# flavie-yuan-liu/DL_attack_on_ImageNet

Hardware: AMD Instinct MI355X
Metric: adversarial images/sec (ADiL learning step, classifier included) (higher is better)
Workload: dtype bf16; 1 GPU; ADiL learn_dictionary_a step vs resnet50, 512 images/GPU, 50 atoms, 224x224, bf16 image streams + fp32 D/V master, loss=logits, clean pseudo-labels computed once per image and cached (1 fwd + 1 bwd per step; result-neutral, profiles/r03_label_stability.md); global_batch=512, atoms=50, inner_iters=131, parallelism=dp1: images+codes sharded, D replicated, 1 all-reduce(grad_d)/step

## Files before the change

### dl_attack_on_imagenet_amd/_lib.py

```python
import ctypes
import os
from ctypes import c_float, c_int, c_size_t, c_void_p

_PKG = os.path.dirname(os.path.abspath(__file__))
LIBPATH = os.environ.get("ADIL_HIP_LIBRARY") or os.path.join(_PKG, "lib", "libadil_hip.so")

SIGNATURES = {
    "adil_abi_version": (c_int, []),
    "adil_max_atoms": (c_int, []),
    "adil_grad_workspace_bytes": (c_size_t, [c_int, c_int, c_int]),
    "adil_grad_code_rows": (c_int, [c_int]),
    "adil_grad_slab_offset": (c_size_t, [c_int, c_int, c_int]),
    "adil_pack_codes": (c_int, [c_void_p, c_void_p, c_int, c_int, c_void_p, c_void_p, c_void_p, c_int, c_void_p, c_int, c_int,
                                c_void_p]),
    "adil_gather_images": (c_int, [c_void_p, c_int, c_void_p, c_void_p, c_int, c_int, c_int, c_void_p]),
    "adil_spd_inverse": (c_int, [c_void_p, c_int, c_void_p, c_void_p]),
    "adil_synth": (c_int, [c_void_p, c_void_p, c_void_p, c_void_p, c_int, c_int, c_int, c_int, c_float, c_int, c_void_p]),
    "adil_images_to_u8": (c_int, [c_void_p, c_int, c_void_p, c_size_t, c_void_p, c_void_p]),
    "adil_synth_store": (c_int, [c_void_p, c_void_p, c_void_p, c_void_p, c_void_p, c_int, c_int, c_int, c_int, c_float, c_int,
                                 c_void_p]),
    "adil_synth_fp8": (c_int, [c_void_p, c_void_p, c_void_p, c_void_p, c_int, c_int, c_int, c_int, c_float, c_float, c_int,
                               c_void_p]),
    "adil_dict_to_fp8": (c_int, [c_void_p, c_size_t, c_void_p, c_void_p]),
    "adil_adamw_clamp_fp8": (c_int, [c_void_p, c_void_p, c_int, c_void_p, c_void_p, c_size_t, c_float, c_float, c_float,
# ... 15 lines not shown
                                  c_float, c_float, c_float, c_float, c_float, c_void_p, c_void_p, c_float, c_void_p, c_void_p,
                                  c_void_p, c_int, c_int, c_void_p]),
    "adil_atom_l1ball_project": (c_int, [c_void_p, c_int, c_int, c_int, c_float, c_void_p]),
    "adil_l1ball_project": (c_int, [c_void_p, c_int, c_int, c_float, c_void_p]),
    "adil_l2ball_project": (c_int, [c_void_p, c_int, c_int, c_float, c_void_p]),
    "adil_ista_step": (c_int, [c_void_p, c_void_p, c_size_t, c_float, c_float, c_void_p]),
    "adil_atom_workspace_bytes": (c_size_t, [c_int, c_int]),
    "adil_atom_norms": (c_int, [c_void_p, c_int, c_int, c_void_p, c_void_p, c_size_t, c_void_p]),
    "adil_atom_scale": (c_int, [c_void_p, c_int, c_int, c_void_p, c_int, c_void_p]),
    "adil_gram_workspace_bytes": (c_size_t, [c_int, c_int]),
    "adil_gram": (c_int, [c_void_p, c_int, c_int, c_void_p, c_void_p, c_size_t, c_void_p]),
    "adil_dict_rightmul": (c_int, [c_void_p, c_void_p, c_int, c_int, c_void_p, c_void_p]),
    "adil_image_metrics": (c_int, [c_void_p, c_void_p, c_int, c_int, c_int, c_void_p, c_void_p, c_void_p]),
    "adil_affine_act_fwd": (c_int, [c_void_p, c_void_p, c_void_p, c_void_p, c_void_p, c_size_t, c_int, c_int, c_int, c_int,
                                    c_void_p]),
    "adil_affine_act_bwd": (c_int, [c_void_p, c_void_p, c_void_p, c_void_p, c_void_p, c_size_t, c_int, c_int, c_int, c_int,
                                    c_void_p]),
    "adil_stem_conv_fwd": (c_int, [c_void_p, c_int, c_void_p, c_float, c_float, c_float, c_float, c_float, c_float,
                                   c_void_p, c_void_p, c_void_p, c_int, c_int, c_int, c_void_p]),
    "adil_maxpool_fwd": (c_int, [c_void_p, c_void_p, c_void_p, c_int, c_int, c_int, c_int, c_void_p]),
    "adil_stem_pool_bwd": (c_int, [c_void_p, c_void_p, c_void_p, c_void_p, c_void_p, c_int, c_int, c_int, c_int, c_void_p]),
    "adil_pw_conv_fwd": (c_int, [c_void_p, c_void_p, c_void_p, c_void_p, c_void_p, c_void_p, c_int, c_int, c_int, c_int,
                                 c_void_p, c_void_p, c_int, c_int, c_void_p]),
    "adil_pw_conv_bwd": (c_int, [c_void_p, c_void_p, c_void_p, c_void_p, c_void_p, c_void_p, c_void_p, c_int, c_int, c_int,
                                 c_int, c_void_p, c_void_p, c_void_p, c_void_p, c_int, c_int, c_void_p]),
    "adil_pw_conv_bwd_tile": (c_int, [c_void_p, c_void_p, c_void_p, c_void_p, c_void_p, c_void_p, c_void_p, c_int, c_int, c_int,
                                      c_int, c_void_p, c_void_p, c_void_p, c_void_p, c_int, c_int, c_void_p, c_int]),
    "adil_pw_route_policy": (c_int, [c_int]),
    "adil_pw_join_fwd": (c_int, [c_void_p, c_void_p, c_void_p, c_void_p, c_void_p, c_void_p, c_void_p, c_void_p, c_void_p,
                                 c_void_p, c_void_p, c_void_p, c_int, c_int, c_int, c_void_p]),
    "adil_pw_join_bwd": (c_int, [c_void_p, c_void_p, c_void_p, c_void_p, c_void_p, c_void_p, c_void_p, c_void_p, c_void_p,
                                 c_void_p, c_void_p, c_void_p, c_void_p, c_int, c_int, c_int, c_void_p]),
    "adil_conv3x3": (c_int, [c_void_p, c_void_p, c_void_p, c_int, c_int, c_int, c_int, c_int, c_void_p]),
    "adil_conv3x3_s2_fwd": (c_int, [c_void_p, c_void_p, c_void_p, c_int, c_int, c_int, c_int, c_int, c_void_p]),
    "adil_conv3x3_s2_bwd": (c_int, [c_void_p, c_void_p, c_void_p, c_int, c_int, c_int, c_int, c_int, c_void_p]),
    "adil_dw3x3_fwd": (c_int, [c_void_p, c_void_p, c_void_p, c_void_p, c_int, c_int, c_int, c_int, c_int, c_int, c_void_p]),
    "adil_dw3x3_bwd": (c_int, [c_void_p, c_void_p, c_void_p, c_void_p, c_int, c_int, c_int, c_int, c_int, c_int, c_void_p]),
    "adil_pw8_fwd": (c_int, [c_void_p, c_void_p, c_void_p, c_void_p, c_void_p, c_void_p, c_int, c_int, c_int, c_int, c_void_p]),
    "adil_pw8_bwd": (c_int, [c_void_p, c_void_p, c_void_p, c_void_p, c_void_p, c_int, c_int, c_int, c_int, c_void_p]),
    "adil_stem_conv_bwd": (c_int, [c_void_p, c_void_p, c_float, c_float, c_float, c_void_p, c_int, c_int, c_int, c_int,
                                   c_void_p]),
    "adil_first3x3_fwd": (c_int, [c_void_p, c_int, c_void_p, c_float, c_float, c_float, c_float, c_float, c_float,
                                  c_void_p, c_void_p, c_void_p, c_int, c_int, c_int, c_int, c_void_p]),
    "adil_first3x3_bwd": (c_int, [c_void_p, c_void_p, c_void_p, c_void_p, c_float, c_float, c_float, c_void_p, c_int, c_int,
                                  c_int, c_int, c_int, c_void_p]),
    "adil_pool_head_fwd": (c_int, [c_void_p, c_void_p, c_void_p, c_void_p, c_void_p, c_int, c_int, c_int, c_int, c_void_p]),
    "adil_pool_head_bwd": (c_int, [c_void_p, c_void_p, c_void_p, c_void_p, c_int, c_int, c_int, c_int, c_void_p]),
    "adil_dense1x1_fwd": (c_int, [c_void_p, c_void_p, c_void_p, c_void_p, c_void_p, c_void_p, c_void_p, c_int, c_int, c_int,
                                  c_int, c_void_p]),
    "adil_dense1x1_bwd": (c_int, [c_void_p, c_void_p, c_void_p, c_void_p, c_void_p, c_void_p, c_void_p, c_void_p, c_int, c_int,
                                  c_int, c_int, c_void_p]),
    "adil_dense3x3_fwd": (c_int, [c_void_p, c_void_p, c_void_p, c_int, c_int, c_int, c_int, c_int, c_void_p]),
    "adil_dense3x3_bwd": (c_int, [c_void_p, c_void_p, c_void_p, c_int, c_int, c_int, c_int, c_int, c_void_p]),
    "adil_dense1x1_fwd_ld": (c_int, [c_void_p, c_int, c_void_p, c_void_p, c_void_p, c_void_p, c_void_p, c_void_p, c_int, c_int,
                                     c_int, c_int, c_int, c_void_p]),
    "adil_dense1x1_bwd_ld": (c_int, [c_void_p, c_int, c_void_p, c_int, c_void_p, c_void_p, c_void_p, c_int, c_void_p, c_void_p,
                                     c_void_p, c_int, c_int, c_int, c_int, c_int, c_int, c_void_p]),
    "adil_dense3x3_fwd_ld": (c_int, [c_void_p, c_int, c_void_p, c_void_p, c_int, c_int, c_int, c_int, c_int, c_int, c_void_p]),
    "adil_dense3x3_bwd_ld": (c_int, [c_void_p, c_int, c_void_p, c_void_p, c_int, c_int, c_int, c_int, c_int, c_int, c_void_p]),
    "adil_dense_transition_fwd": (c_int, [c_void_p, c_void_p, c_void_p, c_void_p, c_void_p, c_int, c_int, c_int, c_int, c_int,
                                          c_void_p]),
    "adil_dense_transition_bwd": (c_int, [c_void_p, c_int, c_void_p, c_void_p, c_void_p, c_void_p, c_void_p, c_int, c_int,
                                          c_int, c_int, c_int, c_void_p]),
}

ABI_VERSION = 8
# ... 39 lines not shown
```

### dl_attack_on_imagenet_amd/csrc/adil_convs.hip

```cpp
#include <hip/hip_runtime.h>
#include <stdint.h>

#include "adil_common.h"
#include "adil_hip.h"
#include "adil_mfma.h"

namespace {

#define PW_BM 128
#define PW_BK 64
#define PW_LS (PW_BK + 8)
#define PW_PK 512

template <int BN, bool PRO, bool RES>
__global__ __launch_bounds__(256) __attribute__((amdgpu_waves_per_eu(PRO && BN == 128 ? 2 : (RES ? 3 : 4)))) void pw_conv_fwd_kernel(
    const bf16_t* __restrict__ x, const bf16_t* __restrict__ wgt, const float* __restrict__ scale,
    const float* __restrict__ shift, const bf16_t* __restrict__ res, bf16_t* __restrict__ y, int M, int K, int N,
    int relu, int MT, int NT, const float* __restrict__ pscale, const float* __restrict__ pshift, int sub_w, int sub_hw) {
    constexpr int CT = BN / 32;
    constexpr int XCH = PW_BM * PW_BK / 8 / 256;
    constexpr int WCH = BN * PW_BK / 8 / 256;
    constexpr int OS = BN + 8;
    extern __shared__ __attribute__((aligned(16))) unsigned char smem_raw[];
    bf16_t* sx = reinterpret_cast<bf16_t*>(smem_raw);
// ... 715 lines not shown

}

extern "C" int adil_pw_join_fwd(const void* h2raw, const float* pscale2, const float* pshift2, const void* w3,
                                const float* scale3, const float* shift3, const void* res, void* out, const void* w1,
                                const float* scale1, const float* shift1, void* h1, int M, int W, int C, void* stream) {
    ADIL_ENTER();
    if (!h2raw || !pscale2 || !pshift2 || !w3 || !scale3 || !shift3 || !res || !out || !w1 || !scale1 || !shift1 || !h1 ||
        M <= 0 || (W != 64 && W != 128) || C != 4 * W)
        return ADIL_EINVAL;
    const JoinArgs a = {(const bf16_t*)h2raw, nullptr, pscale2, pshift2, (const bf16_t*)w3, scale3, shift3,
                        (const bf16_t*)res, nullptr, (bf16_t*)out, (const bf16_t*)w1, scale1, shift1, nullptr, (bf16_t*)h1,
                        M, C};
    return launch_pw_join_w<false>(a, W, (hipStream_t)stream);
}

extern "C" int adil_pw_join_bwd(const void* g_h1, const void* h1, const float* scale1, const void* wt1, const void* g_out,
                                const void* out, const float* scale3, void* gres, const void* wt3, const void* h2raw,
                                const float* pscale2, const float* pshift2, void* gx, int M, int W, int C, void* stream) {
    ADIL_ENTER();
    if (!g_h1 || !h1 || !scale1 || !wt1 || !g_out || !out || !scale3 || !gres || !wt3 || !h2raw || !pscale2 || !pshift2 ||
        !gx || M <= 0 || (W != 64 && W != 128) || C != 4 * W)
        return ADIL_EINVAL;
    const JoinArgs a = {(const bf16_t*)g_h1, (const bf16_t*)h1, scale1, nullptr, (const bf16_t*)wt1, scale3, nullptr,
                        (const bf16_t*)g_out, (const bf16_t*)out, (bf16_t*)gres, (const bf16_t*)wt3, pscale2, pshift2,
                        (const bf16_t*)h2raw, (bf16_t*)gx, M, C};
    return launch_pw_join_w<true>(a, W, (hipStream_t)stream);
}

namespace {

#define C3_LS 72

template <int BN, int WPX>
__global__ __launch_bounds__(256) __attribute__((amdgpu_waves_per_eu(2))) void conv3x3_kernel(
    const bf16_t* __restrict__ x, const bf16_t* __restrict__ wp, bf16_t* __restrict__ y, int M, int H, int W, int C, int N,
    int MT, int NT) {
    constexpr int C3_BM = WPX * 64;
    constexpr int CTW = BN / 32 / (4 / WPX);
    constexpr int XCHK = (C3_BM + 128) * 8 / 256;
    constexpr int WCH = BN * 8 / 256;
    constexpr int OS = BN + 8;
    extern __shared__ __attribute__((aligned(16))) unsigned char smem_raw[];
    const int NP = C3_BM + 2 * W + 2;
    bf16_t* sx = reinterpret_cast<bf16_t*>(smem_raw);
    const int sx_elems = (NP * C3_LS > C3_BM * OS ? NP * C3_LS : C3_BM * OS);
    bf16_t* sw = sx + ((sx_elems + 7) & ~7);
    const int tid = threadIdx.x, lane = tid & 63, w = tid >> 6, c = lane & 31, h = lane >> 5;
    const int wpx = w % WPX, wch = w / WPX;
    int mt, nt;
    if ((MT & 7) == 0) {
        const int xcd = blockIdx.x & 7, j = blockIdx.x >> 3;
        nt = j % NT;
        mt = (j / NT) * 8 + xcd;
    } else {
        nt = blockIdx.x % NT;
        mt = blockIdx.x / NT;
    }
    const int m0 = mt * C3_BM, n0 = nt * BN;
    const int nci = C >> 6;

    int pl[2];
    unsigned vmask[2];
#pragma unroll
    for (int p = 0; p < 2; ++p) {
        pl[p] = (wpx * 2 + p) * 32 + c;
        const int m = m0 + pl[p];
        const int ww = m % W, hh = (m / W) % H;
        unsigned vm = 0;
#pragma unroll
        for (int t = 0; t < 9; ++t) {
            const int kh = t / 3, kw = t - 3 * kh;
            const bool ok = (m < M) && (hh + kh - 1 >= 0) && (hh + kh - 1 < H) && (ww + kw - 1 >= 0) && (ww + kw - 1 < W);
            vm |= ok ? (1u << t) : 0u;
        }
        vmask[p] = vm;
    }

    u32x4 xr[XCHK], wr[3][WCH];
    auto load_x = [&](int cc) {
#pragma unroll
        for (int i = 0; i < XCHK; ++i) {
            const int q = tid + 256 * i, px = q >> 3, ch = q & 7;
            int gm = m0 - W - 1 + (px < NP ? px : NP - 1);
            gm = gm < 0 ? 0 : (gm >= M ? M - 1 : gm);
            xr[i] = *reinterpret_cast<const u32x4*>(x + (size_t)gm * C + cc * 64 + ch * 8);
        }
    };
    auto store_x = [&]() {
#pragma unroll
        for (int i = 0; i < XCHK; ++i) {
            const int q = tid + 256 * i, px = q >> 3, ch = q & 7;
            if (px < NP) *reinterpret_cast<u32x4*>(sx + px * C3_LS + ch * 8) = xr[i];
        }
    };
    const int nit = nci * 9;
    auto load_w = [&](int it, u32x4 (&r)[WCH]) {
        const int itc = it < nit ? it : nit - 1;
        const int cc = itc / 9, tap = itc - 9 * cc;
#pragma unroll
        for (int i = 0; i < WCH; ++i) {
            const int q = tid + 256 * i, row = q >> 3, ch = q & 7;
            r[i] = *reinterpret_cast<const u32x4*>(wp + ((size_t)(n0 + row) * 9 + tap) * C + cc * 64 + ch * 8);
        }
    };
    auto store_w = [&](int buf, const u32x4 (&r)[WCH]) {
#pragma unroll
        for (int i = 0; i < WCH; ++i) {
            const int q = tid + 256 * i, row = q >> 3, ch = q & 7;
            *reinterpret_cast<u32x4*>(sw + (buf * BN + row) * C3_LS + ch * 8) = r[i];
        }
    };

    f32x16 acc[2][CTW];
#pragma unroll
    for (int p = 0; p < 2; ++p)
#pragma unroll
        for (int ct = 0; ct < CTW; ++ct)
#pragma unroll
            for (int r = 0; r < 16; ++r) acc[p][ct][r] = 0.0f;

    auto tap_body = [&](int it, u32x4 (&rfree)[WCH], const u32x4 (&rnext)[WCH]) {
        const int buf = it & 1;
        const int cc = it / 9, tap = it - 9 * cc;
        const int kh = tap / 3, kw = tap - 3 * kh;
        load_w(it + 3, rfree);
        if (tap == 4 && cc + 1 < nci) load_x(cc + 1);
        const bf16_t* bw = sw + (buf * BN + (wch * CTW) * 32 + c) * C3_LS + 8 * h;
        const int shift = kh * W + kw;
        const bool ok0 = (vmask[0] >> tap) & 1u, ok1 = (vmask[1] >> tap) & 1u;
#pragma unroll
        for (int ks = 0; ks < 4; ++ks) {
            bf16x8 b0 = lds8(sx + (pl[0] + shift) * C3_LS + 16 * ks + 8 * h);
            bf16x8 b1 = lds8(sx + (pl[1] + shift) * C3_LS + 16 * ks + 8 * h);
            u32x4 z0 = __builtin_bit_cast(u32x4, b0), z1 = __builtin_bit_cast(u32x4, b1);
#pragma unroll
            for (int j = 0; j < 4; ++j) { z0[j] = ok0 ? z0[j] : 0u; z1[j] = ok1 ? z1[j] : 0u; }
            b0 = __builtin_bit_cast(bf16x8, z0);
            b1 = __builtin_bit_cast(bf16x8, z1);
#pragma unroll
            for (int ct = 0; ct < CTW; ++ct) {
                const bf16x8 a = lds8(bw + ct * 32 * C3_LS + 16 * ks);
                mma16(acc[0][ct], a, b0);
                mma16(acc[1][ct], a, b1);
            }
        }
        if (it + 1 < nit) store_w(buf ^ 1, rnext);
        if (tap == 8 && cc + 1 < nci) {
            lds_barrier();
            store_x();
        }
        lds_barrier();
    };

    load_x(0);
    load_w(0, wr[0]);
    load_w(1, wr[1]);
    load_w(2, wr[2]);
    store_x();
    store_w(0, wr[0]);
    __syncthreads();
    for (int it = 0; it < nit; it += 3) {
        tap_body(it, wr[0], wr[1]);
        tap_body(it + 1, wr[1], wr[2]);
        tap_body(it + 2, wr[2], wr[0]);
    }
#pragma unroll
    for (int p = 0; p < 2; ++p) {
#pragma unroll
        for (int ct = 0; ct < CTW; ++ct) {
#pragma unroll
            for (int q = 0; q < 4; ++q) {
                u32x2 t;
                t[0] = pack2_bf16(acc[p][ct][4 * q], acc[p][ct][4 * q + 1]);
                t[1] = pack2_bf16(acc[p][ct][4 * q + 2], acc[p][ct][4 * q + 3]);
                *reinterpret_cast<u32x2*>(sx + pl[p] * OS + (wch * CTW + ct) * 32 + 8 * q + 4 * h) = t;
            }
        }
    }
    __syncthreads();
    constexpr int CPP = BN / 8;
#pragma unroll
    for (int i = 0; i < C3_BM * CPP / 256; ++i) {
        const int id = tid + 256 * i, px = id / CPP, ch = id - px * CPP;
        const int mm = m0 + px;
        if (mm < M) *reinterpret_cast<u32x4*>(y + (size_t)mm * N + n0 + ch * 8) = *reinterpret_cast<const u32x4*>(sx + px * OS + ch * 8);
    }
}

template <int BN, int WPX>
int launch_conv3x3(const void* x, const void* wp, void* y, int M, int H, int W, int C, int N, hipStream_t st) {
    constexpr int C3_BM = WPX * 64;
    const int MT = (M + C3_BM - 1) / C3_BM, NT = N / BN;
    const int NP = C3_BM + 2 * W + 2;
    size_t sx_elems = (size_t)NP * C3_LS;
    if (sx_elems < (size_t)C3_BM * (BN + 8)) sx_elems = (size_t)C3_BM * (BN + 8);
    sx_elems = (sx_elems + 7) & ~(size_t)7;
    const size_t lds = (sx_elems + (size_t)2 * BN * C3_LS) * sizeof(bf16_t);
    if (lds > 160 * 1024) return ADIL_EINVAL;
    if (lds > 48 * 1024) {
        const hipError_t e = hipFuncSetAttribute((const void*)conv3x3_kernel<BN, WPX>, hipFuncAttributeMaxDynamicSharedMemorySize,
                                                 (int)lds);
        if (e != hipSuccess) return (int)e;
    }
    hipLaunchKernelGGL((conv3x3_kernel<BN, WPX>), dim3((unsigned)(MT * NT)), dim3(256), lds, st, (const bf16_t*)x,
                       (const bf16_t*)wp, (bf16_t*)y, M, H, W, C, N, MT, NT);
    ADIL_CHECK_LAUNCH();
    return 0;
}

}

extern "C" int adil_conv3x3(const void* x, const void* wp, void* y, int B, int H, int W, int C, int N, void* stream) {
    ADIL_ENTER();
    if (!x || !wp || !y || B <= 0 || H <= 0 || W <= 0 || C <= 0 || N <= 0 || (C % 64) || (N % 64) || W > 63) return ADIL_EINVAL;
    const long long M = (long long)B * H * W;
    if (M > 0x7fffffffLL) return ADIL_EINVAL;
    if (N % 128 == 0) return launch_conv3x3<128, 2>(x, wp, y, (int)M, H, W, C, N, (hipStream_t)stream);
    return launch_conv3x3<64, 4>(x, wp, y, (int)M, H, W, C, N, (hipStream_t)stream);
}

namespace {

#define S2_BM 128

template <int BN, bool BWD>
__global__ __launch_bounds__(256) __attribute__((amdgpu_waves_per_eu(2))) void conv3x3_s2_kernel(
    const bf16_t* __restrict__ src, const bf16_t* __restrict__ wp, bf16_t* __restrict__ dst, int M, int OH, int OW, int K,
    int NO, int MT, int NT) {
    constexpr int CTW = BN / 64;
    constexpr int XCH = S2_BM * 8 / 256;
    constexpr int WCH = BN * 8 / 256;
    constexpr int OS = BN + 8;
    constexpr int PAIR = (S2_BM + BN) * C3_LS;
    constexpr int NCLS = BWD ? 4 : 1;
    static_assert(S2_BM * OS <= PAIR, "the output transpose goes through one idle buffer");
    extern __shared__ __attribute__((aligned(16))) unsigned char smem_raw[];
    bf16_t* sb = reinterpret_cast<bf16_t*>(smem_raw);
    const int tid = threadIdx.x, lane = tid & 63, w = tid >> 6, c = lane & 31, h = lane >> 5;
    const int wpx = w & 1, wch = w >> 1;
    int mt, nt;
    if ((MT & 7) == 0) {
        const int xcd = blockIdx.x & 7, j = blockIdx.x >> 3;
        nt = j % NT;
        mt = (j / NT) * 8 + xcd;
    } else {
        nt = blockIdx.x % NT;
        mt = blockIdx.x / NT;
    }
    const int m0 = mt * S2_BM, n0 = nt * BN;
    const int nci = K >> 6;
    const int nit = nci * 9;
    auto cls_ph = [](int cls) { return BWD ? (cls < 2 ? 1 : 0) : 0; };
    auto cls_pw = [](int cls) { return BWD ? ((cls & 1) ? 0 : 1) : 0; };

    int ctr[XCH];
    unsigned flg[XCH];
#pragma unroll
    for (int i = 0; i < XCH; ++i) {
        const int r = m0 + (tid >> 3) + 32 * i;
        const int rc = r < M ? r : M - 1;
        const int j = rc % OW, ii = (rc / OW) % OH;
        ctr[i] = BWD ? rc : 4 * rc - 2 * j;
        const bool okh = BWD ? (ii + 1 < OH) : (ii > 0), okw = BWD ? (j + 1 < OW) : (j > 0);
        flg[i] = (r < M ? 1u : 0u) | (okh ? 2u : 0u) | (okw ? 4u : 0u);
    }
    struct Tile {
        u32x4 x[XCH], w[WCH];
        unsigned ok;
    };
    int lcls = 0, lcc = 0, la = 0, lb = 0;
    int lph = cls_ph(0), lpw = cls_pw(0), lnth = BWD ? 1 + lph : 3, lntw = BWD ? 1 + lpw : 3;
    auto load_tiles = [&](Tile& t) {
        const int kh = BWD ? (lph ? 2 * la : 1) : la, kw = BWD ? (lpw ? 2 * lb : 1) : lb;
        const int off = BWD ? (kh == 0 ? OW : 0) + (kw == 0 ? 1 : 0) : (kh - 1) * 2 * OW + (kw - 1);
        const unsigned need = 1u | (kh == 0 ? 2u : 0u) | (kw == 0 ? 4u : 0u);
        unsigned okm = 0;
#pragma unroll
        for (int i = 0; i < XCH; ++i) {
            const int ch = tid & 7;
            const bool ok = (flg[i] & need) == need;
            okm |= ok ? (1u << i) : 0u;
            const int srow = ok ? ctr[i] + off : ctr[i];
            t.x[i] = *reinterpret_cast<const u32x4*>(src + (size_t)srow * K + lcc * 64 + ch * 8);
        }
        t.ok = okm;
#pragma unroll
        for (int i = 0; i < WCH; ++i) {
            const int q = tid + 256 * i, row = q >> 3, ch = q & 7;
            t.w[i] = *reinterpret_cast<const u32x4*>(wp + ((size_t)(n0 + row) * 9 + kh * 3 + kw) * K + lcc * 64 + ch * 8);
        }
        if (++lb == lntw) {
            lb = 0;
            if (++la == lnth) {
                la = 0;
                if (++lcc == nci && lcls + 1 < NCLS) {
                    lcc = 0;
                    ++lcls;
                    lph = cls_ph(lcls);
                    lpw = cls_pw(lcls);
                    lnth = 1 + lph;
                    lntw = 1 + lpw;
                }
            }
        }
    };
    auto store_tiles = [&](int buf, const Tile& t) {
        bf16_t* sx = sb + buf * PAIR;
        bf16_t* sw = sx + S2_BM * C3_LS;
#pragma unroll
        for (int i = 0; i < XCH; ++i) {
            const int row = (tid >> 3) + 32 * i, ch = tid & 7;
            u32x4 v = t.x[i];
            const bool ok = (t.ok >> i) & 1u;
#pragma unroll
            for (int j = 0; j < 4; ++j) v[j] = ok ? v[j] : 0u;
            *reinterpret_cast<u32x4*>(sx + row * C3_LS + ch * 8) = v;
        }
#pragma unroll
        for (int i = 0; i < WCH; ++i) {
            const int q = tid + 256 * i, row = q >> 3, ch = q & 7;
            *reinterpret_cast<u32x4*>(sw + row * C3_LS + ch * 8) = t.w[i];
        }
    };
// ... 11 lines not shown
    auto finish_class = [&](int cls, bf16_t* so) {
#pragma unroll
        for (int p = 0; p < 2; ++p) {
            const int pl = wpx * 64 + p * 32 + c;
#pragma unroll
            for (int ct = 0; ct < CTW; ++ct) {
#pragma unroll
                for (int q = 0; q < 4; ++q) {
                    u32x2 t;
                    t[0] = pack2_bf16(acc[p][ct][4 * q], acc[p][ct][4 * q + 1]);
                    t[1] = pack2_bf16(acc[p][ct][4 * q + 2], acc[p][ct][4 * q + 3]);
                    *reinterpret_cast<u32x2*>(so + pl * OS + (wch * CTW + ct) * 32 + 8 * q + 4 * h) = t;
                }
            }
        }
        lds_barrier();
        const int ph = cls_ph(cls), pw = cls_pw(cls);
        constexpr int CPP = BN / 8;
#pragma unroll
        for (int i = 0; i < S2_BM * CPP / 256; ++i) {
            const int id = tid + 256 * i, px = id / CPP, ch = id - px * CPP;
            const int r = m0 + px;
            if (r < M) {
                const size_t drow = BWD ? (size_t)(4 * r - 2 * (r % OW) + ph * 2 * OW + pw) : (size_t)r;
                *reinterpret_cast<u32x4*>(dst + drow * NO + n0 + ch * 8) = *reinterpret_cast<const u32x4*>(so + px * OS + ch * 8);
            }
        }
        lds_barrier();
        zero_acc();
    };

    int ccls = 0;
    int crem = nci * (BWD ? 4 : 9);
    auto tap_body = [&](int it, Tile& tfree, const Tile& tnext) {
        const int buf = it & 1;
        if (it + 3 < nit) load_tiles(tfree);
        const bf16_t* bx = sb + buf * PAIR + (wpx * 64 + c) * C3_LS + 8 * h;
        const bf16_t* bw = sb + buf * PAIR + (S2_BM + wch * CTW * 32 + c) * C3_LS + 8 * h;
#pragma unroll
        for (int ks = 0; ks < 4; ++ks) {
            const bf16x8 b0 = lds8(bx + 16 * ks);
            const bf16x8 b1 = lds8(bx + 32 * C3_LS + 16 * ks);
#pragma unroll
            for (int ct = 0; ct < CTW; ++ct) {
                const bf16x8 a = lds8(bw + ct * 32 * C3_LS + 16 * ks);
                mma16(acc[0][ct], a, b0);
                mma16(acc[1][ct], a, b1);
            }
        }
        if (--crem == 0) {
            finish_class(ccls, sb + (buf ^ 1) * PAIR);
            ++ccls;
            crem = nci * (1 + cls_ph(ccls)) * (1 + cls_pw(ccls));
        }
        if (it + 1 < nit) store_tiles(buf ^ 1, tnext);
        lds_barrier();
    };

    Tile t0, t1, t2;
    load_tiles(t0);
    load_tiles(t1);
    load_tiles(t2);
    store_tiles(0, t0);
    lds_barrier();
    for (int it = 0; it < nit; it += 3) {
        tap_body(it, t0, t1);
        tap_body(it + 1, t1, t2);
        tap_body(it + 2, t2, t0);
    }
}

template <int BN, bool BWD>
int launch_conv3x3_s2(const void* src, const void* wp, void* dst, int M, int OH, int OW, int K, int NO, hipStream_t st) {
    const int MT = (M + S2_BM - 1) / S2_BM, NT = NO / BN;
    const size_t lds = (size_t)2 * (S2_BM + BN) * C3_LS * sizeof(bf16_t);
    if (lds > 48 * 1024) {
        const hipError_t e = hipFuncSetAttribute((const void*)conv3x3_s2_kernel<BN, BWD>,
                                                 hipFuncAttributeMaxDynamicSharedMemorySize, (int)lds);
        if (e != hipSuccess) return (int)e;
    }
    hipLaunchKernelGGL((conv3x3_s2_kernel<BN, BWD>), dim3((unsigned)(MT * NT)), dim3(256), lds, st,
                       (const bf16_t*)src, (const bf16_t*)wp, (bf16_t*)dst, M, OH, OW, K, NO, MT, NT);
    ADIL_CHECK_LAUNCH();
    return 0;
}

bool conv3x3_s2_covers(int B, int H, int W, int C, int N, int* M) {
    if (B <= 0 || H <= 0 || W <= 0 || C <= 0 || N <= 0 || (H & 1) || (W & 1) || (C % 64) || (N % 64) || W > ADIL_CONV3X3_S2_MAX_W)
        return false;
    const long long m4 = (long long)B * H * W;
    if (m4 > 0x7fffffffLL) return false;
    *M = (int)(m4 / 4);
    return true;
}

}

extern "C" int adil_conv3x3_s2_fwd(const void* x, const void* wp, void* y, int B, int H, int W, int C, int N, void* stream) {
    ADIL_ENTER();
    int M = 0;
    if (!x || !wp || !y || !conv3x3_s2_covers(B, H, W, C, N, &M)) return ADIL_EINVAL;
    if (N % 128 == 0) return launch_conv3x3_s2<128, false>(x, wp, y, M, H / 2, W / 2, C, N, (hipStream_t)stream);
    return launch_conv3x3_s2<64, false>(x, wp, y, M, H / 2, W / 2, C, N, (hipStream_t)stream);
}

extern "C" int adil_conv3x3_s2_bwd(const void* g, const void* wp_bwd, void* gx, int B, int H, int W, int C, int N, void* stream) {
    ADIL_ENTER();
    int M = 0;
    if (!g || !wp_bwd || !gx || !conv3x3_s2_covers(B, H, W, C, N, &M)) return ADIL_EINVAL;
    if (C % 128 == 0) return launch_conv3x3_s2<128, true>(g, wp_bwd, gx, M, H / 2, W / 2, N, C, (hipStream_t)stream);
    return launch_conv3x3_s2<64, true>(g, wp_bwd, gx, M, H / 2, W / 2, N, C, (hipStream_t)stream);
}
```

### dl_attack_on_imagenet_amd/ops.py

```python
from __future__ import annotations

import math
from ctypes import byref, c_int, c_void_p
from dataclasses import dataclass
from typing import Optional, Tuple

import torch

from . import _lib

Tensor = torch.Tensor
_DTYPE_CODE = {torch.float32: 0, torch.bfloat16: 1}
ADIL_U8 = 2
_workspaces = {}


def _round_up(x: int, m: int) -> int:
    return (x + m - 1) // m * m


def stream_dtype_code(dtype: torch.dtype) -> int:
    try:
        return _DTYPE_CODE[dtype]
    except KeyError:
# ... 780 lines not shown
    @staticmethod
    def backward(ctx, g):
        lib = _lib.load()
        (wp_bwd,) = ctx.saved_tensors
        (c,) = ctx.meta
        g2 = _nhwc_grad(g)
        b, h, w, n = g2.shape
        gx = torch.empty((b, h, w, c), dtype=torch.bfloat16, device=g2.device)
        if b > 0:
            _lib.check(lib.adil_conv3x3(_ptr(g2), _ptr(wp_bwd), _ptr(gx), b, h, w, n, c, _stream()), "adil_conv3x3")
        return gx.permute(0, 3, 1, 2), None, None


def conv3x3(x: Tensor, wp_fwd: Tensor, wp_bwd: Tensor) -> Tensor:
    return Conv3x3Function.apply(x, wp_fwd, wp_bwd)


CONV3X3_S2_MAX_W = 63


def pack_conv3x3_s2_weights(weight: Tensor) -> Tuple[Tensor, Tensor]:
    n, c, kh, kw = weight.shape
    if (kh, kw) != (3, 3):
        raise ValueError(f"expected a 3x3 convolution weight, got {tuple(weight.shape)}")
    w = weight.detach().float()
    fwd = w.permute(0, 2, 3, 1).reshape(n, 9 * c).to(torch.bfloat16).contiguous()
    bwd = w.permute(1, 2, 3, 0).reshape(c, 9 * n).to(torch.bfloat16).contiguous()
    return fwd, bwd


def conv3x3_s2_covers(x: Tensor, cin: int, cout: int) -> bool:
    return (x.dim() == 4 and x.is_cuda and x.dtype == torch.bfloat16 and x.shape[1] == cin and cin % 64 == 0
            and cout % 64 == 0 and x.shape[2] % 2 == 0 and x.shape[3] % 2 == 0 and 0 < x.shape[3] <= CONV3X3_S2_MAX_W
            and x.shape[2] > 0 and x.shape[0] * x.shape[2] * x.shape[3] < 2 ** 31)


class Conv3x3S2Function(torch.autograd.Function):

    @staticmethod
    def forward(ctx, x, wp_fwd, wp_bwd):
        lib = _lib.load()
        b, c, h, w = x.shape
        n = wp_fwd.shape[0]
        x2 = _nhwc(x)
        y = torch.empty((b, h // 2, w // 2, n), dtype=torch.bfloat16, device=x.device)
        if b > 0:
            _lib.check(lib.adil_conv3x3_s2_fwd(_ptr(x2), _ptr(wp_fwd), _ptr(y), b, h, w, c, n, _stream()),
                       "adil_conv3x3_s2_fwd")
        ctx.save_for_backward(wp_bwd)
        ctx.meta = (c, h, w)
        return y.permute(0, 3, 1, 2)

    @staticmethod
    def backward(ctx, g):
        lib = _lib.load()
        (wp_bwd,) = ctx.saved_tensors
        c, h, w = ctx.meta
        g2 = _nhwc_grad(g)
        b, n = g2.shape[0], g2.shape[3]
        gx = torch.empty((b, h, w, c), dtype=torch.bfloat16, device=g2.device)
        if b > 0:
            _lib.check(lib.adil_conv3x3_s2_bwd(_ptr(g2), _ptr(wp_bwd), _ptr(gx), b, h, w, c, n, _stream()),
                       "adil_conv3x3_s2_bwd")
        return gx.permute(0, 3, 1, 2), None, None


def conv3x3_s2(x: Tensor, wp_fwd: Tensor, wp_bwd: Tensor) -> Tensor:
# ... 594 lines not shown
```

### include/adil_hip.h

```cpp
#ifndef ADIL_HIP_H
#define ADIL_HIP_H

#include <stddef.h>
#include <stdint.h>

#ifdef __cplusplus
extern "C" {
#endif

#define ADIL_F32 0
#define ADIL_BF16 1
#define ADIL_U8 2

#define ADIL_EINVAL (-1)
#define ADIL_EWORKSPACE (-2)

int adil_abi_version(void);

int adil_max_atoms(void);

size_t adil_grad_workspace_bytes(int B, int P, int K);

int adil_grad_code_rows(int K);

// ... 61 lines not shown
size_t adil_gram_workspace_bytes(int P, int K);
int adil_gram(const float* d, int P, int K, float* gram, void* ws, size_t ws_bytes, void* stream);

int adil_spd_inverse(const float* a, int K, float* out, void* stream);

int adil_dict_rightmul(const float* d, const float* mat, int P, int K, float* out, void* stream);

int adil_image_metrics(const void* adv, const void* x, int B, int P, int dtype, float* sq_err, float* sq_norm,
                       void* stream);

int adil_affine_act_fwd(const void* x, const void* res, const float* scale, const float* shift, void* y, size_t n, int C,
                        int inner, int relu, int dtype, void* stream);
int adil_affine_act_bwd(const void* g, const void* y, const float* scale, void* gx, void* gres, size_t n, int C,
                        int inner, int relu, int dtype, void* stream);

int adil_stem_conv_fwd(const void* x, int x_dtype, const void* w_fwd, float mean0, float mean1, float mean2, float inv_std0,
                       float inv_std1, float inv_std2, const float* scale, const float* shift, void* y, int B, int H, int W,
                       void* stream);
int adil_maxpool_fwd(const void* y, void* p, uint8_t* idx, int B, int OH, int OW, int C, void* stream);
int adil_stem_pool_bwd(const void* g, const uint8_t* idx, const void* p, const float* scale, void* gy, int B, int OH, int OW,
                       int C, void* stream);
int adil_stem_conv_bwd(const void* gy, const void* w_bwd, float inv_std0, float inv_std1, float inv_std2, void* gx,
                       int gx_dtype, int B, int H, int W, void* stream);

int adil_pw_conv_fwd(const void* x, const void* w, const float* scale, const float* shift, const void* res, void* y, int M,
                     int K, int N, int relu, const float* pscale, const float* pshift, int sub_w, int sub_hw, void* stream);
int adil_pw_conv_bwd(const void* g, const void* g2, const void* y, const float* scale, const void* wt, void* gx, void* gres,
                     int M, int K, int N, int relu, const void* xin, const float* pscale, const float* pshift, const void* g3,
                     int sub_w, int sub_hw, void* stream);
int adil_pw_conv_bwd_tile(const void* g, const void* g2, const void* y, const float* scale, const void* wt, void* gx,
                          void* gres, int M, int K, int N, int relu, const void* xin, const float* pscale,
                          const float* pshift, const void* g3, int sub_w, int sub_hw, void* stream, int bo);
int adil_pw_route_policy(int policy);

int adil_pw_join_fwd(const void* h2raw, const float* pscale2, const float* pshift2, const void* w3, const float* scale3,
                     const float* shift3, const void* res, void* out, const void* w1, const float* scale1,
                     const float* shift1, void* h1, int M, int W, int C, void* stream);
int adil_pw_join_bwd(const void* g_h1, const void* h1, const float* scale1, const void* wt1, const void* g_out,
                     const void* out, const float* scale3, void* gres, const void* wt3, const void* h2raw,
                     const float* pscale2, const float* pshift2, void* gx, int M, int W, int C, void* stream);

int adil_conv3x3(const void* x, const void* wp, void* y, int B, int H, int W, int C, int N, void* stream);

#define ADIL_CONV3X3_S2_MAX_W 63
int adil_conv3x3_s2_fwd(const void* x, const void* wp, void* y, int B, int H, int W, int C, int N, void* stream);
int adil_conv3x3_s2_bwd(const void* g, const void* wp_bwd, void* gx, int B, int H, int W, int C, int N, void* stream);

int adil_dw3x3_fwd(const void* x, const float* w, const float* bias, void* y, int B, int H, int W, int C, int stride,
                   int relu6, void* stream);
int adil_dw3x3_bwd(const void* g, const void* y, const float* w, void* gx, int B, int H, int W, int C, int stride,
                   int relu6, void* stream);

int adil_pw8_fwd(const void* x, const void* w, const float* scale, const float* shift, const void* res, void* y, int M,
                 int K, int N, int act, void* stream);
int adil_pw8_bwd(const void* g, const void* y, const float* scale, const void* wt, void* gx, int M, int K, int N, int act,
                 void* stream);

int adil_first3x3_fwd(const void* x, int x_dtype, const void* w_fwd, float mean0, float mean1, float mean2, float inv_std0,
                      float inv_std1, float inv_std2, const float* scale, const float* shift, void* y, int B, int H, int W,
                      int relu6, void* stream);
int adil_first3x3_bwd(const void* g, const void* y, const float* scale, const void* w_bwd, float inv_std0, float inv_std1,
                      float inv_std2, void* gx, int gx_dtype, int B, int H, int W, int relu6, void* stream);

int adil_pool_head_fwd(const void* x, const float* wt, const float* bias, float* pooled, float* logits, int B, int HW,
                       int C, int N, void* stream);
int adil_pool_head_bwd(const float* g, const float* w, float* gpooled, void* gx, int B, int HW, int C, int N, void* stream);
// ... 30 lines not shown
```

Baseline: 24420 images/sec.

## Software-pipeline LDS fragment reads against MFMA in 3x3 conv main loops

Adds a new default main loop (LOOP=0) for the stride-1 and stride-2 3x3 conv kernels. It double-buffers LDS fragment reads so the next k-slice is read while MFMAs run on the current one, with sched_barrier fences to pin the order. Global loads now use precomputed 32-bit byte offsets, and out-of-image taps point at a zeroed LDS row instead of masking registers. The old loop stays selectable through a new adil_conv3x3_loop switch. The new path adds a 9*C*N overflow guard and one extra LDS row, and the fixed schedule raises register pressure.

```diff
diff --git a/dl_attack_on_imagenet_amd/_lib.py b/dl_attack_on_imagenet_amd/_lib.py
--- a/dl_attack_on_imagenet_amd/_lib.py
+++ b/dl_attack_on_imagenet_amd/_lib.py
@@ -71,6 +71,7 @@
     "adil_pw_join_bwd": (c_int, [c_void_p, c_void_p, c_void_p, c_void_p, c_void_p, c_void_p, c_void_p, c_void_p, c_void_p,
                                  c_void_p, c_void_p, c_void_p, c_void_p, c_int, c_int, c_int, c_void_p]),
     "adil_conv3x3": (c_int, [c_void_p, c_void_p, c_void_p, c_int, c_int, c_int, c_int, c_int, c_void_p]),
+    "adil_conv3x3_loop": (c_int, [c_int]),
     "adil_conv3x3_s2_fwd": (c_int, [c_void_p, c_void_p, c_void_p, c_int, c_int, c_int, c_int, c_int, c_void_p]),
     "adil_conv3x3_s2_bwd": (c_int, [c_void_p, c_void_p, c_void_p, c_int, c_int, c_int, c_int, c_int, c_void_p]),
     "adil_dw3x3_fwd": (c_int, [c_void_p, c_void_p, c_void_p, c_void_p, c_int, c_int, c_int, c_int, c_int, c_int, c_void_p]),
diff --git a/dl_attack_on_imagenet_amd/csrc/adil_convs.hip b/dl_attack_on_imagenet_amd/csrc/adil_convs.hip
--- a/dl_attack_on_imagenet_amd/csrc/adil_convs.hip
+++ b/dl_attack_on_imagenet_amd/csrc/adil_convs.hip
@@ -771,7 +771,7 @@
 
 #define C3_LS 72
 
-template <int BN, int WPX>
+template <int BN, int WPX, int LOOP>
 __global__ __launch_bounds__(256) __attribute__((amdgpu_waves_per_eu(2))) void conv3x3_kernel(
     const bf16_t* __restrict__ x, const bf16_t* __restrict__ wp, bf16_t* __restrict__ y, int M, int H, int W, int C, int N,
     int MT, int NT) {
@@ -817,7 +817,7 @@
     }
 
     u32x4 xr[XCHK], wr[3][WCH];
-    auto load_x = [&](int cc) {
+    [[maybe_unused]] auto load_x = [&](int cc) {
 #pragma unroll
         for (int i = 0; i < XCHK; ++i) {
             const int q = tid + 256 * i, px = q >> 3, ch = q & 7;
@@ -834,7 +834,7 @@
         }
     };
     const int nit = nci * 9;
-    auto load_w = [&](int it, u32x4 (&r)[WCH]) {
+    [[maybe_unused]] auto load_w = [&](int it, u32x4 (&r)[WCH]) {
         const int itc = it < nit ? it : nit - 1;
         const int cc = itc / 9, tap = itc - 9 * cc;
 #pragma unroll
@@ -859,50 +859,153 @@
 #pragma unroll
             for (int r = 0; r < 16; ++r) acc[p][ct][r] = 0.0f;
 
-    auto tap_body = [&](int it, u32x4 (&rfree)[WCH], const u32x4 (&rnext)[WCH]) {
-        const int buf = it & 1;
-        const int cc = it / 9, tap = it - 9 * cc;
-        const int kh = tap / 3, kw = tap - 3 * kh;
-        load_w(it + 3, rfree);
-        if (tap == 4 && cc + 1 < nci) load_x(cc + 1);
-        const bf16_t* bw = sw + (buf * BN + (wch * CTW) * 32 + c) * C3_LS + 8 * h;
-        const int shift = kh * W + kw;
-        const bool ok0 = (vmask[0] >> tap) & 1u, ok1 = (vmask[1] >> tap) & 1u;
-#pragma unroll
-        for (int ks = 0; ks < 4; ++ks) {
-            bf16x8 b0 = lds8(sx + (pl[0] + shift) * C3_LS + 16 * ks + 8 * h);
-            bf16x8 b1 = lds8(sx + (pl[1] + shift) * C3_LS + 16 * ks + 8 * h);
-            u32x4 z0 = __builtin_bit_cast(u32x4, b0), z1 = __builtin_bit_cast(u32x4, b1);
-#pragma unroll
-            for (int j = 0; j < 4; ++j) { z0[j] = ok0 ? z0[j] : 0u; z1[j] = ok1 ? z1[j] : 0u; }
-            b0 = __builtin_bit_cast(bf16x8, z0);
-            b1 = __builtin_bit_cast(bf16x8, z1);
+    if constexpr (LOOP == 1) {
+        auto tap_body = [&](int it, u32x4 (&rfree)[WCH], const u32x4 (&rnext)[WCH]) {
+            const int buf = it & 1;
+            const int cc = it / 9, tap = it - 9 * cc;
+            const int kh = tap / 3, kw = tap - 3 * kh;
+            load_w(it + 3, rfree);
+            if (tap == 4 && cc + 1 < nci) load_x(cc + 1);
+            const bf16_t* bw = sw + (buf * BN + (wch * CTW) * 32 + c) * C3_LS + 8 * h;
+            const int shift = kh * W + kw;
+            const bool ok0 = (vmask[0] >> tap) & 1u, ok1 = (vmask[1] >> tap) & 1u;
+#pragma unroll
+            for (int ks = 0; ks < 4; ++ks) {
+                bf16x8 b0 = lds8(sx + (pl[0] + shift) * C3_LS + 16 * ks + 8 * h);
+                bf16x8 b1 = lds8(sx + (pl[1] + shift) * C3_LS + 16 * ks + 8 * h);
+                u32x4 z0 = __builtin_bit_cast(u32x4, b0), z1 = __builtin_bit_cast(u32x4, b1);
+#pragma unroll
+                for (int j = 0; j < 4; ++j) { z0[j] = ok0 ? z0[j] : 0u; z1[j] = ok1 ? z1[j] : 0u; }
+                b0 = __builtin_bit_cast(bf16x8, z0);
+                b1 = __builtin_bit_cast(bf16x8, z1);
+#pragma unroll
+                for (int ct = 0; ct < CTW; ++ct) {
+                    const bf16x8 a = lds8(bw + ct * 32 * C3_LS + 16 * ks);
+                    mma16(acc[0][ct], a, b0);
+                    mma16(acc[1][ct], a, b1);
+                }
+            }
+            if (it + 1 < nit) store_w(buf ^ 1, rnext);
+            if (tap == 8 && cc + 1 < nci) {
+                lds_barrier();
+                store_x();
+            }
+            lds_barrier();
+        };
+
+        load_x(0);
+        load_w(0, wr[0]);
+        load_w(1, wr[1]);
+        load_w(2, wr[2]);
+        store_x();
+        store_w(0, wr[0]);
+        __syncthreads();
+        for (int it = 0; it < nit; it += 3) {
+            tap_body(it, wr[0], wr[1]);
+            tap_body(it + 1, wr[1], wr[2]);
+            tap_body(it + 2, wr[2], wr[0]);
+        }
+    } else {
+        const unsigned wq = (((unsigned)(n0 + (tid >> 3)) * 9u) * (unsigned)C + (unsigned)(tid & 7) * 8u) * 2u;
+        const size_t wrow = (size_t)32 * 9 * C;
+        auto load_w0 = [&](unsigned ws, u32x4 (&r)[WCH]) {
+#pragma unroll
+            for (int i = 0; i < WCH; ++i)
+                r[i] = *reinterpret_cast<const u32x4*>(reinterpret_cast<const char*>(wp + ws + i * wrow) + wq);
+        };
+        const int gmb = m0 - W - 1 > 0 ? m0 - W - 1 : 0;
+        const bf16_t* xb = x + (size_t)gmb * C;
+        unsigned xq[XCHK];
+#pragma unroll
+        for (int i = 0; i < XCHK; ++i) {
+            const int px = (tid >> 3) + 32 * i;
+            int gm = m0 - W - 1 + (px < NP ? px : NP - 1);
+            gm = gm < 0 ? 0 : (gm >= M ? M - 1 : gm);
+            xq[i] = ((unsigned)(gm - gmb) * (unsigned)C + (unsigned)(tid & 7) * 8u) * 2u;
+        }
+        auto load_x0 = [&](int cc) {
+#pragma unroll
+            for (int i = 0; i < XCHK; ++i)
+                xr[i] = *reinterpret_cast<const u32x4*>(reinterpret_cast<const char*>(xb + cc * 64) + xq[i]);
+        };
+        bf16_t* sz = sw + 2 * BN * C3_LS;
+        const bf16_t* xl0 = sx + pl[0] * C3_LS + 8 * h;
+        const bf16_t* xl1 = sx + pl[1] * C3_LS + 8 * h;
+        const bf16_t* zl = sz + 8 * h;
+        const bf16_t* bwl = sw + ((wch * CTW) * 32 + c) * C3_LS + 8 * h;
+        auto xrow = [&](const bf16_t* xl, unsigned vm, int tap) -> const bf16_t* {
+            const int kh = tap / 3, kw = tap - 3 * kh;
+            const bf16_t* a = xl + (kh * W + kw) * C3_LS;
+            if (tap == 4) return a;
+            return (vm & (1u << tap)) ? a : zl;
+        };
+        struct Frag {
+            bf16x8 b0, b1, a[CTW];
+        };
+        auto read_frag = [&](Frag& f, const bf16_t* p0, const bf16_t* p1, const bf16_t* bw, int ks) {
+            f.b0 = lds8(p0 + 16 * ks);
+            f.b1 = lds8(p1 + 16 * ks);
+#pragma unroll
+            for (int ct = 0; ct < CTW; ++ct) f.a[ct] = lds8(bw + ct * 32 * C3_LS + 16 * ks);
+        };
+        auto mma_frag = [&](const Frag& f) {
 #pragma unroll
             for (int ct = 0; ct < CTW; ++ct) {
-                const bf16x8 a = lds8(bw + ct * 32 * C3_LS + 16 * ks);
-                mma16(acc[0][ct], a, b0);
-                mma16(acc[1][ct], a, b1);
-            }
-        }
-        if (it + 1 < nit) store_w(buf ^ 1, rnext);
-        if (tap == 8 && cc + 1 < nci) {
-            lds_barrier();
-            store_x();
-        }
-        lds_barrier();
-    };
-
-    load_x(0);
-    load_w(0, wr[0]);
-    load_w(1, wr[1]);
-    load_w(2, wr[2]);
-    store_x();
-    store_w(0, wr[0]);
-    __syncthreads();
-    for (int it = 0; it < nit; it += 3) {
-        tap_body(it, wr[0], wr[1]);
-        tap_body(it + 1, wr[1], wr[2]);
-        tap_body(it + 2, wr[2], wr[0]);
+                mma16(acc[0][ct], f.a[ct], f.b0);
+                mma16(acc[1][ct], f.a[ct], f.b1);
+            }
+        };
+
+        load_x0(0);
+        load_w0(0u, wr[0]);
+        load_w0((unsigned)C, wr[1]);
+        load_w0(2u * (unsigned)C, wr[2]);
+        store_x();
+        store_w(0, wr[0]);
+        if (tid < C3_LS / 8) reinterpret_cast<u32x4*>(sz)[tid] = u32x4{0u, 0u, 0u, 0u};
+        __syncthreads();
+        Frag fa, fb;
+        const bf16_t* p0 = xrow(xl0, vmask[0], 0);
+        const bf16_t* p1 = xrow(xl1, vmask[1], 0);
+        read_frag(fa, p0, p1, bwl, 0);
+        for (int cc = 0; cc < nci; ++cc) {
+            const bool more = cc + 1 < nci;
+            const unsigned wsc = (unsigned)cc * 64u, wsn = (unsigned)(more ? cc + 1 : cc) * 64u;
+#pragma unroll
+            for (int tap = 0; tap < 9; ++tap) {
+                const int buf = (cc + tap) & 1;
+                const bf16_t* bw = bwl + buf * BN * C3_LS;
+                const bool last = !more && tap == 8;
+                read_frag(fb, p0, p1, bw, 1);
+                if (!last) store_w(buf ^ 1, wr[(tap + 1) % 3]);
+                load_w0(tap + 3 < 9 ? wsc + (unsigned)((tap + 3) * C) : wsn + (unsigned)((tap - 6) * C), wr[tap % 3]);
+                if (tap == 4 && more) load_x0(cc + 1);
+                __builtin_amdgcn_sched_barrier(0);
+                mma_frag(fa);
+                __builtin_amdgcn_sched_barrier(0);
+                read_frag(fa, p0, p1, bw, 2);
+                __builtin_amdgcn_sched_barrier(0);
+                mma_frag(fb);
+                __builtin_amdgcn_sched_barrier(0);
+                read_frag(fb, p0, p1, bw, 3);
+                __builtin_amdgcn_sched_barrier(0);
+                mma_frag(fa);
+                __builtin_amdgcn_sched_barrier(0);
+                lds_barrier();
+                if (tap == 8 && more) {
+                    store_x();
+                    lds_barrier();
+                }
+                if (!last) {
+                    p0 = xrow(xl0, vmask[0], (tap + 1) % 9);
+                    p1 = xrow(xl1, vmask[1], (tap + 1) % 9);
+                    read_frag(fa, p0, p1, bwl + (buf ^ 1) * BN * C3_LS, 0);
+                }
+                __builtin_amdgcn_sched_barrier(0);
+                mma_frag(fb);
+                __builtin_amdgcn_sched_barrier(0);
+            }
+        }
     }
 #pragma unroll
     for (int p = 0; p < 2; ++p) {
@@ -927,7 +1030,7 @@
     }
 }
 
-template <int BN, int WPX>
+template <int BN, int WPX, int LOOP>
 int launch_conv3x3(const void* x, const void* wp, void* y, int M, int H, int W, int C, int N, hipStream_t st) {
     constexpr int C3_BM = WPX * 64;
     const int MT = (M + C3_BM - 1) / C3_BM, NT = N / BN;
@@ -935,19 +1038,27 @@
     size_t sx_elems = (size_t)NP * C3_LS;
     if (sx_elems < (size_t)C3_BM * (BN + 8)) sx_elems = (size_t)C3_BM * (BN + 8);
     sx_elems = (sx_elems + 7) & ~(size_t)7;
-    const size_t lds = (sx_elems + (size_t)2 * BN * C3_LS) * sizeof(bf16_t);
+    const size_t lds = (sx_elems + (size_t)2 * BN * C3_LS + (LOOP == 0 ? C3_LS : 0)) * sizeof(bf16_t);
     if (lds > 160 * 1024) return ADIL_EINVAL;
     if (lds > 48 * 1024) {
-        const hipError_t e = hipFuncSetAttribute((const void*)conv3x3_kernel<BN, WPX>, hipFuncAttributeMaxDynamicSharedMemorySize,
-                                                 (int)lds);
+        const hipError_t e = hipFuncSetAttribute((const void*)conv3x3_kernel<BN, WPX, LOOP>,
+                                                 hipFuncAttributeMaxDynamicSharedMemorySize, (int)lds);
         if (e != hipSuccess) return (int)e;
     }
-    hipLaunchKernelGGL((conv3x3_kernel<BN, WPX>), dim3((unsigned)(MT * NT)), dim3(256), lds, st, (const bf16_t*)x,
+    hipLaunchKernelGGL((conv3x3_kernel<BN, WPX, LOOP>), dim3((unsigned)(MT * NT)), dim3(256), lds, st, (const bf16_t*)x,
                        (const bf16_t*)wp, (bf16_t*)y, M, H, W, C, N, MT, NT);
     ADIL_CHECK_LAUNCH();
     return 0;
 }
 
+static int g_conv3x3_loop = 0;
+
+}
+
+extern "C" int adil_conv3x3_loop(int variant) {
+    const int prev = g_conv3x3_loop;
+    if (variant == 0 || variant == 1) g_conv3x3_loop = variant;
+    return prev;
 }
 
 extern "C" int adil_conv3x3(const void* x, const void* wp, void* y, int B, int H, int W, int C, int N, void* stream) {
@@ -955,15 +1066,21 @@
     if (!x || !wp || !y || B <= 0 || H <= 0 || W <= 0 || C <= 0 || N <= 0 || (C % 64) || (N % 64) || W > 63) return ADIL_EINVAL;
     const long long M = (long long)B * H * W;
     if (M > 0x7fffffffLL) return ADIL_EINVAL;
-    if (N % 128 == 0) return launch_conv3x3<128, 2>(x, wp, y, (int)M, H, W, C, N, (hipStream_t)stream);
-    return launch_conv3x3<64, 4>(x, wp, y, (int)M, H, W, C, N, (hipStream_t)stream);
+    if (9LL * C * N > 0x7fffffffLL) return ADIL_EINVAL;
+    const hipStream_t st = (hipStream_t)stream;
+    if (g_conv3x3_loop == 1) {
+        if (N % 128 == 0) return launch_conv3x3<128, 2, 1>(x, wp, y, (int)M, H, W, C, N, st);
+        return launch_conv3x3<64, 4, 1>(x, wp, y, (int)M, H, W, C, N, st);
+    }
+    if (N % 128 == 0) return launch_conv3x3<128, 2, 0>(x, wp, y, (int)M, H, W, C, N, st);
+    return launch_conv3x3<64, 4, 0>(x, wp, y, (int)M, H, W, C, N, st);
 }
 
 namespace {
 
 #define S2_BM 128
 
-template <int BN, bool BWD>
+template <int BN, bool BWD, int LOOP>
 __global__ __launch_bounds__(256) __attribute__((amdgpu_waves_per_eu(2))) void conv3x3_s2_kernel(
     const bf16_t* __restrict__ src, const bf16_t* __restrict__ wp, bf16_t* __restrict__ dst, int M, int OH, int OW, int K,
     int NO, int MT, int NT) {
@@ -973,6 +1090,7 @@
     constexpr int OS = BN + 8;
     constexpr int PAIR = (S2_BM + BN) * C3_LS;
     constexpr int NCLS = BWD ? 4 : 1;
+    constexpr bool PIPE = LOOP == 0 && BN == 64;
     static_assert(S2_BM * OS <= PAIR, "the output transpose goes through one idle buffer");
     extern __shared__ __attribute__((aligned(16))) unsigned char smem_raw[];
     bf16_t* sb = reinterpret_cast<bf16_t*>(smem_raw);
@@ -1010,25 +1128,45 @@
     };
     int lcls = 0, lcc = 0, la = 0, lb = 0;
     int lph = cls_ph(0), lpw = cls_pw(0), lnth = BWD ? 1 + lph : 3, lntw = BWD ? 1 + lpw : 3;
+    size_t sq[XCH];
+#pragma unroll
+    for (int i = 0; i < XCH; ++i) sq[i] = ((size_t)ctr[i] * K + (tid & 7) * 8) * sizeof(bf16_t);
+    const unsigned wq = (((unsigned)(n0 + (tid >> 3)) * 9u) * (unsigned)K + (unsigned)(tid & 7) * 8u) * 2u;
+    const size_t wrow = (size_t)32 * 9 * K;
     auto load_tiles = [&](Tile& t) {
         const int kh = BWD ? (lph ? 2 * la : 1) : la, kw = BWD ? (lpw ? 2 * lb : 1) : lb;
         const int off = BWD ? (kh == 0 ? OW : 0) + (kw == 0 ? 1 : 0) : (kh - 1) * 2 * OW + (kw - 1);
         const unsigned need = 1u | (kh == 0 ? 2u : 0u) | (kw == 0 ? 4u : 0u);
         unsigned okm = 0;
-#pragma unroll
-        for (int i = 0; i < XCH; ++i) {
-            const int ch = tid & 7;
-            const bool ok = (flg[i] & need) == need;
-            okm |= ok ? (1u << i) : 0u;
-            const int srow = ok ? ctr[i] + off : ctr[i];
-            t.x[i] = *reinterpret_cast<const u32x4*>(src + (size_t)srow * K + lcc * 64 + ch * 8);
+        if constexpr (LOOP == 1) {
+#pragma unroll
+            for (int i = 0; i < XCH; ++i) {
+                const int ch = tid & 7;
+                const bool ok = (flg[i] & need) == need;
+                okm |= ok ? (1u << i) : 0u;
+                const int srow = ok ? ctr[i] + off : ctr[i];
+                t.x[i] = *reinterpret_cast<const u32x4*>(src + (size_t)srow * K + lcc * 64 + ch * 8);
+            }
+#pragma unroll
+            for (int i = 0; i < WCH; ++i) {
+                const int q = tid + 256 * i, row = q >> 3, ch = q & 7;
+                t.w[i] = *reinterpret_cast<const u32x4*>(wp + ((size_t)(n0 + row) * 9 + kh * 3 + kw) * K + lcc * 64 + ch * 8);
+            }
+        } else {
+            const char* sbase = reinterpret_cast<const char*>(src + lcc * 64);
+            const long long toff = (long long)off * K * (long long)sizeof(bf16_t);
+#pragma unroll
+            for (int i = 0; i < XCH; ++i) {
+                const bool ok = (flg[i] & need) == need;
+                okm |= ok ? (1u << i) : 0u;
+                t.x[i] = *reinterpret_cast<const u32x4*>(sbase + sq[i] + (ok ? toff : 0LL));
+            }
+            const bf16_t* wbase = wp + (kh * 3 + kw) * K + lcc * 64;
+#pragma unroll
+            for (int i = 0; i < WCH; ++i)
+                t.w[i] = *reinterpret_cast<const u32x4*>(reinterpret_cast<const char*>(wbase + i * wrow) + wq);
         }
         t.ok = okm;
-#pragma unroll
-        for (int i = 0; i < WCH; ++i) {
-            const int q = tid + 256 * i, row = q >> 3, ch = q & 7;
-            t.w[i] = *reinterpret_cast<const u32x4*>(wp + ((size_t)(n0 + row) * 9 + kh * 3 + kw) * K + lcc * 64 + ch * 8);
-        }
         if (++lb == lntw) {
             lb = 0;
             if (++la == lnth) {
@@ -1106,7 +1244,7 @@
 
     int ccls = 0;
     int crem = nci * (BWD ? 4 : 9);
-    auto tap_body = [&](int it, Tile& tfree, const Tile& tnext) {
+    [[maybe_unused]] auto tap_body = [&](int it, Tile& tfree, const Tile& tnext) {
         const int buf = it & 1;
         if (it + 3 < nit) load_tiles(tfree);
         const bf16_t* bx = sb + buf * PAIR + (wpx * 64 + c) * C3_LS + 8 * h;
@@ -1129,6 +1267,53 @@
         }
         if (it + 1 < nit) store_tiles(buf ^ 1, tnext);
         lds_barrier();
+    };
+
+    struct Frag {
+        bf16x8 b0, b1, a[CTW];
+    };
+    auto read_frag = [&](Frag& f, int buf, int ks) {
+        const bf16_t* bx = sb + buf * PAIR + (wpx * 64 + c) * C3_LS + 8 * h;
+        const bf16_t* bw = sb + buf * PAIR + (S2_BM + wch * CTW * 32 + c) * C3_LS + 8 * h;
+        f.b0 = lds8(bx + 16 * ks);
+        f.b1 = lds8(bx + 32 * C3_LS + 16 * ks);
+#pragma unroll
+        for (int ct = 0; ct < CTW; ++ct) f.a[ct] = lds8(bw + ct * 32 * C3_LS + 16 * ks);
+    };
+    auto mma_frag = [&](const Frag& f) {
+#pragma unroll
+        for (int ct = 0; ct < CTW; ++ct) {
+            mma16(acc[0][ct], f.a[ct], f.b0);
+            mma16(acc[1][ct], f.a[ct], f.b1);
+        }
+    };
+    Frag fa, fb;
+    [[maybe_unused]] auto tap_body0 = [&](int it, Tile& tfree, const Tile& tnext) {
+        const int buf = it & 1;
+        read_frag(fb, buf, 1);
+        if (it + 1 < nit) store_tiles(buf ^ 1, tnext);
+        if (it + 3 < nit) load_tiles(tfree);
+        __builtin_amdgcn_sched_barrier(0);
+        mma_frag(fa);
+        __builtin_amdgcn_sched_barrier(0);
+        read_frag(fa, buf, 2);
+        __builtin_amdgcn_sched_barrier(0);
+        mma_frag(fb);
+        __builtin_amdgcn_sched_barrier(0);
+        read_frag(fb, buf, 3);
+        __builtin_amdgcn_sched_barrier(0);
+        mma_frag(fa);
+        __builtin_amdgcn_sched_barrier(0);
+        lds_barrier();
+        if (it + 1 < nit) read_frag(fa, buf ^ 1, 0);
+        __builtin_amdgcn_sched_barrier(0);
+        mma_frag(fb);
+        __builtin_amdgcn_sched_barrier(0);
+        if (--crem == 0) {
+            finish_class(ccls, sb + buf * PAIR);
+            ++ccls;
+            crem = nci * (1 + cls_ph(ccls)) * (1 + cls_pw(ccls));
+        }
     };
 
     Tile t0, t1, t2;
@@ -1137,26 +1322,41 @@
     load_tiles(t2);
     store_tiles(0, t0);
     lds_barrier();
-    for (int it = 0; it < nit; it += 3) {
-        tap_body(it, t0, t1);
-        tap_body(it + 1, t1, t2);
-        tap_body(it + 2, t2, t0);
-    }
-}
-
-template <int BN, bool BWD>
-int launch_conv3x3_s2(const void* src, const void* wp, void* dst, int M, int OH, int OW, int K, int NO, hipStream_t st) {
+    if constexpr (!PIPE) {
+        for (int it = 0; it < nit; it += 3) {
+            tap_body(it, t0, t1);
+            tap_body(it + 1, t1, t2);
+            tap_body(it + 2, t2, t0);
+        }
+    } else {
+        read_frag(fa, 0, 0);
+        for (int it = 0; it < nit; it += 3) {
+            tap_body0(it, t0, t1);
+            tap_body0(it + 1, t1, t2);
+            tap_body0(it + 2, t2, t0);
+        }
+    }
+}
+
+template <int BN, bool BWD, int LOOP>
+int launch_conv3x3_s2_loop(const void* src, const void* wp, void* dst, int M, int OH, int OW, int K, int NO, hipStream_t st) {
     const int MT = (M + S2_BM - 1) / S2_BM, NT = NO / BN;
     const size_t lds = (size_t)2 * (S2_BM + BN) * C3_LS * sizeof(bf16_t);
     if (lds > 48 * 1024) {
-        const hipError_t e = hipFuncSetAttribute((const void*)conv3x3_s2_kernel<BN, BWD>,
+        const hipError_t e = hipFuncSetAttribute((const void*)conv3x3_s2_kernel<BN, BWD, LOOP>,
                                                  hipFuncAttributeMaxDynamicSharedMemorySize, (int)lds);
         if (e != hipSuccess) return (int)e;
     }
-    hipLaunchKernelGGL((conv3x3_s2_kernel<BN, BWD>), dim3((unsigned)(MT * NT)), dim3(256), lds, st,
+    hipLaunchKernelGGL((conv3x3_s2_kernel<BN, BWD, LOOP>), dim3((unsigned)(MT * NT)), dim3(256), lds, st,
                        (const bf16_t*)src, (const bf16_t*)wp, (bf16_t*)dst, M, OH, OW, K, NO, MT, NT);
     ADIL_CHECK_LAUNCH();
     return 0;
+}
+
+template <int BN, bool BWD>
+int launch_conv3x3_s2(const void* src, const void* wp, void* dst, int M, int OH, int OW, int K, int NO, hipStream_t st) {
+    if (g_conv3x3_loop == 1) return launch_conv3x3_s2_loop<BN, BWD, 1>(src, wp, dst, M, OH, OW, K, NO, st);
+    return launch_conv3x3_s2_loop<BN, BWD, 0>(src, wp, dst, M, OH, OW, K, NO, st);
 }
 
 bool conv3x3_s2_covers(int B, int H, int W, int C, int N, int* M) {
@@ -1164,6 +1364,7 @@
         return false;
     const long long m4 = (long long)B * H * W;
     if (m4 > 0x7fffffffLL) return false;
+    if (9LL * C * N > 0x7fffffffLL) return false;
     *M = (int)(m4 / 4);
     return true;
 }
diff --git a/dl_attack_on_imagenet_amd/ops.py b/dl_attack_on_imagenet_amd/ops.py
--- a/dl_attack_on_imagenet_amd/ops.py
+++ b/dl_attack_on_imagenet_amd/ops.py
@@ -836,7 +836,7 @@
 def conv3x3_s2_covers(x: Tensor, cin: int, cout: int) -> bool:
     return (x.dim() == 4 and x.is_cuda and x.dtype == torch.bfloat16 and x.shape[1] == cin and cin % 64 == 0
             and cout % 64 == 0 and x.shape[2] % 2 == 0 and x.shape[3] % 2 == 0 and 0 < x.shape[3] <= CONV3X3_S2_MAX_W
-            and x.shape[2] > 0 and x.shape[0] * x.shape[2] * x.shape[3] < 2 ** 31)
+            and x.shape[2] > 0 and x.shape[0] * x.shape[2] * x.shape[3] < 2 ** 31 and 9 * cin * cout < 2 ** 31)
 
 
 class Conv3x3S2Function(torch.autograd.Function):
diff --git a/include/adil_hip.h b/include/adil_hip.h
--- a/include/adil_hip.h
+++ b/include/adil_hip.h
@@ -117,6 +117,7 @@
                           void* gres, int M, int K, int N, int relu, const void* xin, const float* pscale,
                           const float* pshift, const void* g3, int sub_w, int sub_hw, void* stream, int bo);
 int adil_pw_route_policy(int policy);
+int adil_conv3x3_loop(int variant);
 
 int adil_pw_join_fwd(const void* h2raw, const float* pscale2, const float* pshift2, const void* w3, const float* scale3,
                      const float* shift3, const void* res, void* out, const void* w1, const float* scale1,
```

New measurement: 25260 images/sec, median of 6. +3.4%, better.
